# araju6/parameter-server-distributed

Hardware: AMD Instinct MI355X
Metric: samples/sec (whole node) ResNet-50 async-SGD (higher is better)
Workload: dtype bf16

## Files before the change

### parameter_server_distributed_amd/csrc/kernels/convn.hip

```cpp
#include "mfma_common.h"
#include "cu_count.h"
#include "launchers_convn.h"

namespace psd {

namespace {

constexpr int kBM = 128;
constexpr int kBK = 64;

__device__ __forceinline__ bf16x8 frag(const uint8_t* lds, int rb, int ks, int lane) {
  const int row = rb * 16 + (lane & 15);
  return __builtin_bit_cast(bf16x8, *reinterpret_cast<const u32x4*>(lds + kmaj_off(row, ks * 4 + (lane >> 4))));
}

template <int DPSK, int A, int OFF = 0>
__device__ __forceinline__ void wait_ahead(int ahead) {
  if constexpr (A <= 0) {
    wait_vm<OFF>();
  } else {
    if (ahead >= A) wait_vm<A * DPSK + OFF>();
    else wait_ahead<DPSK, A - 1, OFF>(ahead);
  }
}
// ... 835 lines not shown
        pf_at = T;
        __builtin_amdgcn_sched_barrier(0);
      } else {
        convn_epilogue<BM, BN, WNT, STATS, BWD, true>(a, acc, kshift, tile, wr, wc, lane, stg, pix, n0, es);
      }
#pragma unroll
      for (int i = 0; i < 4; ++i)
#pragma unroll
        for (int j = 0; j < G::JN; ++j) acc[i][j] = f32x4{0.f, 0.f, 0.f, 0.f};
    }
  }
  convn_flush<WNT, STATS, BWD>(a, es, (int64_t)blockIdx.x * G::WM + wr, wc, lane, n0);
}

__device__ __forceinline__ int hx_swz(int row) { return ((row >> 1) & 3) << 1; }
__device__ __forceinline__ int hx_off(int row, int kc) { return row * 128 + ((kc ^ hx_swz(row)) << 4); }

constexpr int kHxWin = 4 * 64 * 128;
constexpr int kHxW = 9 * 64 * 128;
constexpr int kHxLds = kHxW + 2 * kHxWin + 4 * 2048 + 512;

template <bool STATS, int BWD>
__global__ __launch_bounds__(256) void convh_kernel(ConvnArgs a, int ntiles) {
  extern __shared__ __attribute__((aligned(16))) uint8_t smem[];
  uint8_t* wlds = smem;
  auto winb = [&](int b) { return smem + kHxW + b * kHxWin; };
  const int lane = threadIdx.x & 63;
  const int wid = __builtin_amdgcn_readfirstlane(threadIdx.x >> 6);
  const int wr = wid >> 1, wc = wid & 1;
  const int cl = lane & 15;
  const int tpi = (a.Ho + 1) >> 1;
  const int t_begin = (int)(((int64_t)blockIdx.x * ntiles) / gridDim.x);
  const int t_end = (int)(((int64_t)(blockIdx.x + 1) * ntiles) / gridDim.x);
  if (t_begin >= t_end) return;
  float kshift[2] = {0.f, 0.f};
  if constexpr (STATS) {
#pragma unroll
    for (int j = 0; j < 2; ++j) kshift[j] = a.shift[wc * 32 + j * 16 + cl];
  }
  const rsrc_t xr = make_rsrc(a.x, a.xbytes);
  const rsrc_t wrs = make_rsrc(a.w, a.wbytes);
  for (int pc = wid; pc < 72; pc += 4) {
    const int t = pc >> 3, row = (pc & 7) * 8 + (lane >> 3);
    const int kc = (lane & 7) ^ hx_swz(row);
    const uint32_t off = ((uint32_t)row * (uint32_t)a.K + (uint32_t)(t * 64 + kc * 8)) * 2u;
    __builtin_amdgcn_raw_ptr_buffer_load_lds(wrs, (__attribute__((address_space(3))) void*)(wlds + pc * 1024), 16, off,
                                             0, 0, 0);
  }
  auto stage = [&](int tile, int b) {
    const int n = tile / tpi, ho0 = (tile - n * tpi) * 2;
#pragma unroll
    for (int i = 0; i < 8; ++i) {
      const int pc = i * 4 + wid;
      const int row = pc * 8 + (lane >> 3);
      const int jj = row >> 6, ws = row & 63;
      const int hi = ho0 - 1 + jj, wi = ws - 1;
      const int kc = (lane & 7) ^ hx_swz(row);
      const bool ok = (unsigned)hi < (unsigned)a.H && (unsigned)wi < (unsigned)a.W;
      const uint32_t off = ok ? ((((uint32_t)((n * a.H + hi) * a.W + wi)) << 6) + (uint32_t)(kc * 8)) * 2u : kOOB;
      __builtin_amdgcn_raw_ptr_buffer_load_lds(xr, (__attribute__((address_space(3))) void*)(winb(b) + pc * 1024), 16,
                                               off, 0, 0, 0);
    }
  };
  stage(t_begin, 0);
  wait_vm<0>();
  __syncthreads();
  uint8_t* stg = smem + kHxW + 2 * kHxWin + wid * 2048;
  EpiSums<2> es;
  es.zero();
  auto pix_of = [&](int tl) {
    const int n = tl / tpi, ho0 = (tl - n * tpi) * 2;
    return [=](int p) -> int {
      const int j = p >> 6, wo = p & 63;
      return ((wo < a.Wo) & (ho0 + j < a.Ho)) ? (n * a.Ho + ho0 + j) * a.Wo + wo : -1;
    };
  };
  for (int tile = t_begin, it = 0; tile < t_end; ++tile, ++it) {
    const int b = it & 1;
    if (tile + 1 < t_end) stage(tile + 1, b ^ 1);
    const uint8_t* win = winb(b);
    f32x4 acc[4][2];
#pragma unroll
    for (int i = 0; i < 4; ++i)
#pragma unroll
      for (int j = 0; j < 2; ++j) acc[i][j] = f32x4{0.f, 0.f, 0.f, 0.f};
    auto load_tap = [&](int tap, bf16x8 (&af)[2][4], bf16x8 (&bf)[2][2]) {
      const int tr = tap / 3, ts = tap - tr * 3;
      const uint8_t* Bs = wlds + tap * 8192;
#pragma unroll
      for (int ks = 0; ks < 2; ++ks) {
#pragma unroll
        for (int j = 0; j < 2; ++j)
          bf[ks][j] = __builtin_bit_cast(
              bf16x8, *reinterpret_cast<const u32x4*>(Bs + hx_off((wc * 2 + j) * 16 + (lane & 15), ks * 4 + (lane >> 4))));
#pragma unroll
        for (int i = 0; i < 4; ++i) {
          const int row = (wr + tr) * 64 + i * 16 + (lane & 15) + ts;
          af[ks][i] = __builtin_bit_cast(bf16x8, *reinterpret_cast<const u32x4*>(win + hx_off(row, ks * 4 + (lane >> 4))));
        }
      }
    };
    bf16x8 fa[2][2][4], fb[2][2][2];
    load_tap(0, fa[0], fb[0]);
#pragma unroll
    for (int tap = 0; tap < 9; ++tap) {
      const int cb = tap & 1;
      if (tap + 1 < 9) load_tap(tap + 1, fa[cb ^ 1], fb[cb ^ 1]);
      __builtin_amdgcn_sched_barrier(0);
#pragma unroll
      for (int ks = 0; ks < 2; ++ks)
#pragma unroll
        for (int i = 0; i < 4; ++i)
#pragma unroll
          for (int j = 0; j < 2; ++j)
            acc[i][j] = __builtin_amdgcn_mfma_f32_16x16x32_bf16(fa[cb][ks][i], fb[cb][ks][j], acc[i][j], 0, 0, 0);
      __builtin_amdgcn_sched_barrier(0);
    }
    wait_vm<0>();
    convn_epilogue<128, 64, 32, STATS, BWD, true>(a, acc, kshift, tile, wr, wc, lane, stg, pix_of(tile), 0, es);
    __syncthreads();
  }
  convn_flush<32, STATS, BWD>(a, es, (int64_t)blockIdx.x * 2 + wr, wc, lane, 0);
}

static bool convh_ok(const ConvnArgs& a) {
  return a.N == 64 && a.logC == 6 && a.R == 3 && a.S == 3 && a.stride == 1 && a.pad == 1 && a.H == a.Ho &&
         a.W == a.Wo && a.Wo + 2 <= 64 && !a.x2 && a.K == 576 && a.ldc == 64;
}

static int convh_grid(int ntiles) { return ntiles < cu_count() ? ntiles : cu_count(); }

template <bool STATS, int BWD>
static hipError_t convh_launch_t(const ConvnArgs& a, hipStream_t st) {
  static bool attr = false;
  if (!attr) {
    const hipError_t e =
        hipFuncSetAttribute((const void*)convh_kernel<STATS, BWD>, hipFuncAttributeMaxDynamicSharedMemorySize, kHxLds);
    if (e != hipSuccess) return e;
    attr = true;
  }
  const int ntiles = (a.M / (a.Ho * a.Wo)) * ((a.Ho + 1) / 2);
  hipLaunchKernelGGL((convh_kernel<STATS, BWD>), dim3(convh_grid(ntiles)), dim3(256), kHxLds, st, a, ntiles);
  return hipGetLastError();
}

static hipError_t convh_launch(const ConvnArgs& a, hipStream_t st) {
  if (a.bwd == 1) return convh_launch_t<false, 1>(a, st);
  if (a.bwd == 2) return convh_launch_t<false, 2>(a, st);
  if (a.bwd == 3) return convh_launch_t<false, 3>(a, st);
  if (a.bwd == 5) return convh_launch_t<false, 5>(a, st);
  return a.part ? convh_launch_t<true, 0>(a, st) : convh_launch_t<false, 0>(a, st);
}

template <int BN>
struct P1Cfg;
template <>
struct P1Cfg<256> {
  static constexpr int WNT = 64;
};
template <>
struct P1Cfg<128> {
  static constexpr int WNT = 32;
};
template <>
struct P1Cfg<64> {
  static constexpr int WNT = 32;
};
constexpr int kP1Slots = 3;
template <int BN>
constexpr int p1_lds() {
  using G = Geo<128, BN, P1Cfg<BN>::WNT, kP1Slots>;
  return kP1Slots * G::SLOT + G::NW * G::STG;
}

static int convp_grid_x(int tiles_m, int tiles_n) {
  int g = cu_count() / (tiles_n > 0 ? tiles_n : 1);
  if (g < 1) g = 1;
  return g < tiles_m ? g : tiles_m;
}

template <int BN>
static bool pf_ok(const ConvnArgs& a) {
  return BN == 256 && a.epi_prefetch && (a.bwd == 2 || a.bwd == 5 || a.bwd == 8) && a.ldc == a.N &&
         (int64_t)a.M * a.N * 2 <= 0xFFFFFF00ll && a.M < (1 << 24);
}

template <int BN, bool STATS, int BWD, bool PF = false, bool HASBX = true>
static hipError_t convp_launch_t(const ConvnArgs& a0, hipStream_t st, int grid_mul = 1) {
  constexpr int WNT = P1Cfg<BN>::WNT;
  using G = Geo<128, BN, WNT, kP1Slots>;
  constexpr int LDS = p1_lds<BN>();
  static_assert(LDS <= 160 * 1024, "LDS");
  static bool attr = false;
  if (!attr) {
    const hipError_t e = hipFuncSetAttribute((const void*)convp_kernel<BN, WNT, kP1Slots, STATS, BWD, PF, HASBX>,
                                             hipFuncAttributeMaxDynamicSharedMemorySize, LDS);
    if (e != hipSuccess) return e;
    attr = true;
  }
  ConvnArgs a = a0;
  a.nslot = kP1Slots;
  const int tiles_m = (a.M + 127) / 128, tiles_n = a.N / BN;
  int gx = convp_grid_x(tiles_m, tiles_n) * grid_mul;
  if (gx > tiles_m) gx = tiles_m;
  hipLaunchKernelGGL((convp_kernel<BN, WNT, kP1Slots, STATS, BWD, PF, HASBX>), dim3(gx, tiles_n), dim3(G::NT), LDS, st,
                     a, tiles_m);
  return hipGetLastError();
}

template <int BN>
static int pr_slots(int K) {
  using G = Geo<128, BN, P1Cfg<BN>::WNT, 3>;
  const int fixed = (K / kBK) * BN * 128 + G::NW * G::STG;
  int ns = (160 * 1024 - fixed) / (128 * 128);
  if (ns > kPrMaxSlots) ns = kPrMaxSlots;
  return ns >= 3 ? ns : 0;
}

template <int BN, bool STATS, int BWD, bool PF = false, bool HASBX = true>
static hipError_t convpr_launch_t(const ConvnArgs& a0, int ns, hipStream_t st, int grid_mul = 1) {
  constexpr int WNT = P1Cfg<BN>::WNT;
  using G = Geo<128, BN, WNT, 3>;
  static bool attr = false;
  if (!attr) {
    const hipError_t e = hipFuncSetAttribute((const void*)convpr_kernel<BN, WNT, STATS, BWD, PF, HASBX>,
                                             hipFuncAttributeMaxDynamicSharedMemorySize, 160 * 1024);
    if (e != hipSuccess) return e;
    attr = true;
  }
  ConvnArgs a = a0;
  a.nslot = ns;
  const int lds = (a.K / kBK) * BN * 128 + ns * 128 * 128 + G::NW * G::STG;
  const int tiles_m = (a.M + 127) / 128, tiles_n = a.N / BN;
  int gx = convp_grid_x(tiles_m, tiles_n) * grid_mul;
  if (gx > tiles_m) gx = tiles_m;
  hipLaunchKernelGGL((convpr_kernel<BN, WNT, STATS, BWD, PF, HASBX>), dim3(gx, tiles_n), dim3(G::NT), lds, st, a,
                     tiles_m);
  return hipGetLastError();
}

template <int BN>
static hipError_t convpr_launch_s(const ConvnArgs& a, int ns, hipStream_t st, int gm = 1) {
  if constexpr (BN == 256) {
    if (pf_ok<BN>(a)) {
      const bool hb = a.bx != nullptr;
      if (a.bwd == 2) return hb ? convpr_launch_t<BN, false, 2, true, true>(a, ns, st, gm)
                                : convpr_launch_t<BN, false, 2, true, false>(a, ns, st, gm);
      if (a.bwd == 5) return hb ? convpr_launch_t<BN, false, 5, true, true>(a, ns, st, gm)
                                : convpr_launch_t<BN, false, 5, true, false>(a, ns, st, gm);
      if (a.bwd == 8) return convpr_launch_t<BN, false, 8, true, true>(a, ns, st, gm);
    }
  }
  if (a.bwd == 1) return convpr_launch_t<BN, false, 1>(a, ns, st, gm);
  if (a.bwd == 2) return convpr_launch_t<BN, false, 2>(a, ns, st, gm);
  if (a.bwd == 3) return convpr_launch_t<BN, false, 3>(a, ns, st, gm);
  if (a.bwd == 5) return convpr_launch_t<BN, false, 5>(a, ns, st, gm);
  if (a.bwd == 8) return convpr_launch_t<BN, false, 8>(a, ns, st, gm);
  return a.part ? convpr_launch_t<BN, true, 0>(a, ns, st, gm) : convpr_launch_t<BN, false, 0>(a, ns, st, gm);
}

template <int BN>
static hipError_t convp_launch_s(const ConvnArgs& a, hipStream_t st, int gm = 1) {
  if (const int ns = pr_slots<BN>(a.K)) return convpr_launch_s<BN>(a, ns, st, gm);
  if constexpr (BN == 256) {
    if (pf_ok<BN>(a)) {
      const bool hb = a.bx != nullptr;
      if (a.bwd == 2) return hb ? convp_launch_t<BN, false, 2, true, true>(a, st, gm)
                                : convp_launch_t<BN, false, 2, true, false>(a, st, gm);
      if (a.bwd == 5) return hb ? convp_launch_t<BN, false, 5, true, true>(a, st, gm)
                                : convp_launch_t<BN, false, 5, true, false>(a, st, gm);
      if (a.bwd == 8) return convp_launch_t<BN, false, 8, true, true>(a, st, gm);
    }
  }
  if (a.bwd == 1) return convp_launch_t<BN, false, 1>(a, st, gm);
  if (a.bwd == 2) return convp_launch_t<BN, false, 2>(a, st, gm);
  if (a.bwd == 3) return convp_launch_t<BN, false, 3>(a, st, gm);
  if (a.bwd == 5) return convp_launch_t<BN, false, 5>(a, st, gm);
  if (a.bwd == 8) return convp_launch_t<BN, false, 8>(a, st, gm);
  return a.part ? convp_launch_t<BN, true, 0>(a, st, gm) : convp_launch_t<BN, false, 0>(a, st, gm);
}

template <int BN>
static hipError_t convp2_launch_s(const ConvnArgs& a, hipStream_t st) {
  using G = Geo<128, BN, P1Cfg<BN>::WNT, 3>;
  const int lds2 = (a.K / kBK) * BN * 128 + 2 * 128 * 128 + G::NW * G::STG;
  if (lds2 <= 80 * 1024) return convpr_launch_s<BN>(a, 2, st, 2);
  return convp_launch_s<BN>(a, st, 2);
}

static hipError_t convp2_launch(const ConvnArgs& a, int bn, hipStream_t st) {
  if (a.R != 1 || a.S != 1 || a.stride != 1 || a.pad != 0 || a.Ho != a.H || a.Wo != a.W) return hipErrorNotSupported;
  if (bn == 256) return convp2_launch_s<256>(a, st);
  if (bn == 128) return convp2_launch_s<128>(a, st);
  return convp2_launch_s<64>(a, st);
}

static hipError_t convp_launch(const ConvnArgs& a, int bn, hipStream_t st) {
  if (a.R != 1 || a.S != 1 || a.stride != 1 || a.pad != 0 || a.Ho != a.H || a.Wo != a.W) return hipErrorNotSupported;
  if (bn == 256) return convp_launch_s<256>(a, st);
  if (bn == 128) return convp_launch_s<128>(a, st);
  return convp_launch_s<64>(a, st);
}

template <int BM, int BN, int WNT, int NSLOT, bool STATS, int BWD>
static hipError_t convn_launch_t(const ConvnArgs& a0, hipStream_t st) {
  using G = Geo<BM, BN, WNT, NSLOT>;
  constexpr int LDS_MAX = NSLOT * G::SLOT + G::NW * G::STG;
  static_assert(LDS_MAX <= 160 * 1024, "LDS");
  static bool attr = false;
  if (!attr) {
    const hipError_t e = hipFuncSetAttribute((const void*)convn_kernel<BM, BN, WNT, NSLOT, STATS, BWD>,
                                             hipFuncAttributeMaxDynamicSharedMemorySize, LDS_MAX);
    if (e != hipSuccess) return e;
    attr = true;
  }
  ConvnArgs a = a0;
  const int nt = a.K / kBK;
  a.nslot = nt < NSLOT ? (nt < 2 ? 1 : nt) : NSLOT;
  const int lds = a.nslot * G::SLOT + G::NW * G::STG;
  const int tiles_m = (a.M + BM - 1) / BM;
  hipLaunchKernelGGL((convn_kernel<BM, BN, WNT, NSLOT, STATS, BWD>), dim3(tiles_m, a.N / BN), dim3(G::NT), lds, st, a);
  return hipGetLastError();
}

template <int BM, int BN, int WNT, int NSLOT>
static hipError_t convn_launch_s(const ConvnArgs& a, hipStream_t st) {
  if (a.bwd == 1) return convn_launch_t<BM, BN, WNT, NSLOT, false, 1>(a, st);
  if (a.bwd == 2) return convn_launch_t<BM, BN, WNT, NSLOT, false, 2>(a, st);
  if (a.bwd == 3) return convn_launch_t<BM, BN, WNT, NSLOT, false, 3>(a, st);
  if (a.bwd == 5) return convn_launch_t<BM, BN, WNT, NSLOT, false, 5>(a, st);
  if (a.bwd == 8) return convn_launch_t<BM, BN, WNT, NSLOT, false, 8>(a, st);
  return a.part ? convn_launch_t<BM, BN, WNT, NSLOT, true, 0>(a, st)
                : convn_launch_t<BM, BN, WNT, NSLOT, false, 0>(a, st);
}

int convn_tile_n(int N) {
  if (N == 64) return 64;
  if (N == 128) return 128;
  if (N % 256 == 0) return 256;
  return 0;
}

static int plain_count(int bn) { return bn == 256 ? 3 : 4; }
static int persist_count(int bn) { return bn == 64 ? 1 : 0; }
static int p1_count(int bn) { return bn ? 2 : 0; }
static int convn_variant_count(int bn) { return plain_count(bn) + persist_count(bn) + p1_count(bn); }
static bool is_persist(int bn, int v) { return v >= plain_count(bn) && v < plain_count(bn) + persist_count(bn); }
static bool is_p1(int bn, int v) { return v == plain_count(bn) + persist_count(bn); }
static bool is_p2(int bn, int v) { return v == plain_count(bn) + persist_count(bn) + 1; }

int convn_variant_kind(int N, int v) {
  const int bn = convn_tile_n(N);
  if (!bn || v < 0 || v >= convn_variant_count(bn)) return -1;
  return v < plain_count(bn) ? 0 : is_persist(bn, v) ? 2 : is_p1(bn, v) ? 3 : 4;
}

int convn_variants(int N) {
  const int bn = convn_tile_n(N);
  return bn ? convn_variant_count(bn) : 0;
}

static int default_variant(const ConvnArgs& a, int bn) {
  (void)a;
  (void)bn;
  return 0;
}

static int variant_bm(int bn, int v) {
  if (is_persist(bn, v) || is_p1(bn, v) || is_p2(bn, v)) return 128;
  if (bn == 64) return (v == 2 || v == 3) ? 256 : 128;
  if (bn == 128) return v == 2 ? 256 : 128;
  return 128;
}

bool convn_variant_ok(int N, int v, int R, int S, int stride, int pad, int Wo, bool has_x2) {
  const int bn = convn_tile_n(N);
  if (!bn || v < 0 || v >= convn_variant_count(bn)) return false;
  if (v < plain_count(bn)) return true;
  if (is_p1(bn, v) || is_p2(bn, v)) return R == 1 && S == 1 && stride == 1 && pad == 0;
  return !has_x2 && N == 64 && R == 3 && S == 3 && stride == 1 && pad == 1 && Wo + 2 <= 64;
}

int convn_stats_rows(int M) { return 4 * ((M + 255) / 256) + 4; }

int convn_part_rows_geo(int M, int N, int variant, int Ho, int Wo, int R) {
  const int bn = convn_tile_n(N);
  if (!bn) return 0;
  const int bm = variant_bm(bn, variant);
  if (is_persist(bn, variant)) {
    if (Ho <= 0 || Wo <= 0) return 0;
    return 2 * convh_grid((M / (Ho * Wo)) * ((Ho + 1) / 2));
  }
  if (is_p1(bn, variant)) return 2 * convp_grid_x((M + 127) / 128, N / bn);
  if (is_p2(bn, variant)) {
    const int t = (M + 127) / 128, g = 2 * convp_grid_x(t, N / bn);
    return 2 * (g < t ? g : t);
  }
  return (bm / 64) * ((M + bm - 1) / bm);
}

int convn_part_rows(int M, int N, int variant) { return convn_part_rows_geo(M, N, variant, 0, 0, 1); }

hipError_t launch_convn(const ConvnArgs& a_in, hipStream_t st) {
  if (a_in.M <= 0) return hipSuccess;
  ConvnArgs a = a_in;
  if (!a.x2) a.K1 = a.K;
  const int bn = convn_tile_n(a.N);
  const int C = 1 << a.logC;
  const bool two = a.x2 != nullptr;
  const int K1 = two ? a.K1 : a.K;
  const bool ok = bn > 0 && a.logC >= 6 && a.K % kBK == 0 && K1 == a.R * a.S * C && a.ldc % 8 == 0 &&
                  (!two || (a.R == 1 && a.S == 1 && a.stride == 1 && a.pad == 0 && a.logC2 >= 6 && K1 % kBK == 0 &&
                            a.K == K1 + (1 << a.logC2) && a.x2bytes > 0 && a.x2bytes <= 0xFFFFFF00u)) &&
                  a.ldc >= a.N && a.H < 32768 && a.W < 32768 && a.xbytes > 0 && a.xbytes <= 0xFFFFFF00u &&
                  a.wbytes > 0 && a.variant < convn_variant_count(bn) &&
                  (a.y || (a.bwd == 0 && a.part)) &&
                  (a.bwd == 0 ? (!a.part || a.shift)
                   : a.bwd == 8 ? (!a.part && a.bss && a.amask && a.ldc == a.N && a.N % 8 == 0)
                              : (a.part && (a.bx || a.bwd >= 2) && a.bmean && a.ldc == a.N &&
                                 (a.bwd == 1 ? a.bss != nullptr
                                             : ((a.bwd == 2 || a.bwd == 3 || a.bwd == 5) && a.bdr && a.bmbits &&
                                                (a.bwd != 3 || (a.bxd && a.bmean_d && a.part_d)) &&
                                                (a.bwd != 5 || (a.Ho % 2 == 0 && a.Wo % 2 == 0))))));
  if (!ok) return hipErrorNotSupported;
  if (a.ophase != 0 &&
      (a.ophase > 4 || a.variant < 0 || a.variant >= plain_count(bn) || two || a.stride != 1 || a.pad != 0 ||
       (a.bwd != 0 && a.bwd != 1) || a.M >= (1 << 24) || a.R > 2 || a.S > 2 ||
       (int64_t)a.M * 4 * a.ldc * 2 > 0x7FFFFFFFll))
    return hipErrorNotSupported;
  const int v = a.variant >= 0 ? a.variant : default_variant(a, bn);
  if (is_p1(bn, v)) return convp_launch(a, bn, st);
  if (is_p2(bn, v)) return convp2_launch(a, bn, st);
  if (is_persist(bn, v)) {
    if (!convh_ok(a) || a.bwd == 8 || !a.y) return hipErrorNotSupported;
    return convh_launch(a, st);
  }
  switch (bn) {
    case 64:
      if (v == 0) return convn_launch_s<128, 64, 32, 3>(a, st);
      if (v == 1) return convn_launch_s<128, 64, 32, 2>(a, st);
      if (v == 2) return convn_launch_s<256, 64, 64, 3>(a, st);
      return convn_launch_s<256, 64, 32, 3>(a, st);
    case 128:
      if (v == 0) return convn_launch_s<128, 128, 32, 3>(a, st);
      if (v == 1) return convn_launch_s<128, 128, 64, 3>(a, st);
      if (v == 2) return convn_launch_s<256, 128, 64, 2>(a, st);
      return convn_launch_s<128, 128, 32, 2>(a, st);
    default:
      if (v == 0) return convn_launch_s<128, 256, 64, 3>(a, st);
      if (v == 1) return convn_launch_s<128, 256, 64, 2>(a, st);
      return convn_launch_s<128, 128, 32, 2>(a, st);
  }
}

}
```

### parameter_server_distributed_amd/ops/conv.py

```python
from __future__ import annotations


import functools

import torch
import torch.nn as nn
import torch.nn.functional as F

from ..utils.config import feature as _feat
from . import wprep as _wprep
from . import autotune as _at
from .handover import (BwdPre, StatsPending, StridedDr, bn_momentum, fold_v as _fold_v, pop_dr, same, sinks, take,
                       take_dr)


def _enabled() -> bool:
    return _feat("conv1x1")


def _choose(key: tuple, candidates: dict) -> str:
    return _at.choose(("conv1x1",) + key, candidates, "miopen")


def decisions() -> dict:
# ... 5 lines not shown


def _native():
    from .. import native

    return native()


def _psd_ok(k: int, n: int) -> bool:
    return k % 8 == 0 and n % 8 == 0 and _feat("conv1x1_mfma")


def _as_2d(t: torch.Tensor) -> torch.Tensor:
    n, c, h, w = t.shape
    return t.permute(0, 2, 3, 1).reshape(n * h * w, c)


def _from_2d(t2: torch.Tensor, n: int, h: int, w: int) -> torch.Tensor:
    return t2.view(n, h, w, t2.shape[1]).permute(0, 3, 1, 2)


def _fp8_ok(k: int, n: int) -> bool:
    return k % 128 == 0 and k >= 256 and n >= 256 and n % 8 == 0 and _feat("fp8_compute")


def _q8(t2: torch.Tensor, e5m2: bool = False, scaler: "DelayedScale | None" = None):
    from . import quantize_fp8

    if scaler is not None:
        return scaler.quantize(t2, e5m2)
    return quantize_fp8(t2, e5m2=e5m2)


from .fp8_common import FP8_CALLS, mx_weight


def _mx_on() -> bool:
    return _feat("fp8_mx")


def _q_act(t: torch.Tensor, e5m2: bool = False, scaler: "DelayedScale | None" = None):
    if _mx_on():
        from . import quantize_mx

        return quantize_mx(t, e5m2=e5m2)
    return _q8(t, e5m2=e5m2, scaler=scaler)


def _q_weight(mod, w2: torch.Tensor):
    if _mx_on():
        return mx_weight(mod, w2)
    return _q8(w2)


def _take_dq8(mod, dy: torch.Tensor):
    return take(mod, "_psd_dq8_pending", dy, strides=True)


def _take_q8(mod, x: torch.Tensor):
    return take(mod, "_psd_q8_pending", x, strides=True)




def _psdn_ok(cin: int, cout: int) -> bool:
    return cin >= 64 and (cin & (cin - 1)) == 0 and (cout in (64, 128) or cout % 256 == 0) and \
        _feat("convn")


def _bn_consumer(mod):
    bn = getattr(mod, "_psd_bn", None) if mod is not None else None
    if bn is None or not bn.training or bn.running_mean is None or not _feat("convn_stats"):
        return None
    return bn


class _Lazy:
    __slots__ = ("fn", "t", "shape")

    def __init__(self, fn, shape):
        self.fn, self.t, self.shape = fn, None, tuple(shape)

    def __call__(self) -> torch.Tensor:
        if self.t is None:
            self.t = self.fn()
        return self.t


def _wt(w2: torch.Tensor, mod=None, weight=None) -> _Lazy:
    def make():
        t = _wprep.get(mod, weight, "t") if weight is not None else None
        return t if t is not None else w2.t().contiguous()
    return _Lazy(make, (w2.shape[1], w2.shape[0]))


def _wflip(mod, weight: torch.Tensor) -> torch.Tensor:
    t = _wprep.get(mod, weight, "f")
    if t is not None:
        return t
    cout, cin, k, _ = weight.shape
    return weight.flip(2, 3).permute(1, 2, 3, 0).reshape(cin, k * k * cout).contiguous()


def _get(w):
    return w() if isinstance(w, _Lazy) else w


def _out_hw(h: int, w: int, k: int, stride: int, pad: int) -> tuple:
    return (h + 2 * pad - k) // stride + 1, (w + 2 * pad - k) // stride + 1


def _convn_variants(x, w2, k: int, stride: int, pad: int, bn=None) -> dict:
    C = _native()
    n, _, h, w = x.shape
    cout = w2.shape[0]
    ho, wo = _out_hw(h, w, k, stride, pad)
    M = n * ho * wo

    def make(v, stats):
        def fn():
            out = torch.empty(M, cout, device=x.device, dtype=x.dtype)
            part = None
            if stats:
                part = torch.empty(_part_rows(M, cout, v, ho, wo, k), 2, cout, device=x.device, dtype=torch.float32)
            rows = C.convn_(x, _get(w2), out, k, k, stride, pad, part=part,
                            shift=bn.running_mean if stats else None, variant=v)
            if rows == 0:
                raise RuntimeError("convn_ declined a shape _psdn_ok accepted")
            y = _from_2d(out, n, ho, wo)
            if stats:
                bn._psd_stats_pending = StatsPending(y, part, rows)
            return y
        return fn

    ok = [v for v in range(C.convn_variants(cout)) if _variant_ok(cout, v, k, stride, pad, wo, x.shape[1], h)]
    cands = {f"psdn{v}": make(v, bn is not None) for v in ok}
    if bn is not None:
        cands.update({f"psdu{v}": make(v, False) for v in ok})
    return cands


def _variant_ok(cout: int, v: int, k: int, stride: int, pad: int, wo: int, cin: int | None = None,
                h: int | None = None) -> bool:
    C = _native()
    if not C.convn_variant_ok(cout, v, k, k, stride, pad, wo):
        return False
    kind = C.convn_variant_kind(cout, v)
    if kind == 2:
        return _feat("convn_persist") and cin == 64 and (h is None or h == wo)
    if kind == 3:
        return _feat("convn_p1")
    if kind == 4:
        return _feat("convn_p1") and _feat("convn_p2")
    return kind == 0


def _part_rows(M: int, N: int, v: int, ho: int, wo: int, k: int) -> int:
    C = _native()
    return max(C.convn_stats_rows(M), C.convn_part_rows(M, N, v, ho, wo, k))


def _fwd_records(ctx, mod) -> None:
    ctx.bn_in = getattr(mod, "_psd_bn_in", None) if mod is not None else None
    ctx.strided_to = getattr(mod, "_psd_strided_to", None) if mod is not None else None


def _bn_bwd_fusion(bn, x: torch.Tensor):
    st = getattr(bn, "_psd_fwd", None) if bn is not None else None
    if st is None or not _feat("convn_bwd"):
        return None
    y, bx, mean, ss, mbits, xd, mean_d = st
    if not same(y, x, strides=True):
        return None
    if mbits is not None:
        if not bn._psd_pending_dr:
            return None
        if isinstance(bn._psd_pending_dr[-1], StridedDr):
            if xd is not None or x.shape[2] % 2 or x.shape[3] % 2 or not _feat("convn_bwd5"):
                return None
            return dict(mode=5, bn=bn, bx=bx, mean=mean, mbits=mbits)
        if xd is not None:
            if not _feat("convn_bwd3"):
                return None
            return dict(mode=3, bn=bn, bx=bx, mean=mean, mbits=mbits, bxd=xd, mean_d=mean_d)
        return dict(mode=2, bn=bn, bx=bx, mean=mean, mbits=mbits)
    return dict(mode=1, bn=bn, bx=bx, mean=mean, ss=ss)


def _take_dr_for(fu) -> None:
    if fu is not None:
        fu["dr"] = fu["bn"]._psd_pending_dr.pop() if fu["mode"] >= 2 else None


def _convn_bwd_launch(dy, w2, cout: int, k: int, pad: int, v: int, fu: dict, prows: int, declined: str,
                      x2=None, bias=None) -> torch.Tensor:
    n, _, h, w = dy.shape
    out = torch.empty(n * h * w, cout, device=dy.device, dtype=dy.dtype)
    part = torch.empty(prows, 2, cout, device=dy.device, dtype=torch.float32)
    part_d = torch.empty_like(part) if fu["mode"] == 3 else None
    rows = _native().convn_bwd_(dy, w2, out, k, k, 1, pad, part, v, fu["mode"], fu["bx"], fu["mean"],
                                bss=fu.get("ss"), bdr=_dr_arg(fu.get("dr")), bmbits=fu.get("mbits"), x2=x2,
                                bias=bias, bxd=fu.get("bxd"), bmean_d=fu.get("mean_d"), part_d=part_d,
                                epi_prefetch=_feat("convp_epi_prefetch"))
    if rows == 0:
        raise RuntimeError(declined)
    g = _from_2d(out, n, h, w)
    fu["bn"]._psd_bwd_pre = BwdPre(g, part, rows, part_d)
    return g


def _convn_bwd_variants(dy, w2, k: int, pad: int, fu: dict) -> dict:
    C = _native()
    n, _, h, w = dy.shape
    cout = w2.shape[0]

    def make(v):
        return lambda: _convn_bwd_launch(dy, _get(w2), cout, k, pad, v, fu, _part_rows(n * h * w, cout, v, h, w, k) + 1,
                                         "convn_bwd_ declined a shape _psdn_ok accepted")

    return {f"psdnb{v}": make(v) for v in range(C.convn_variants(cout))
            if _variant_ok(cout, v, k, 1, pad, w, dy.shape[1], h)}


def _s2_phase_weights(weight: torch.Tensor) -> list:
    cin = weight.shape[1]
    sel = (lambda t, d: t.narrow(d, 1, 1), lambda t, d: t[(slice(None),) * d + (slice(None, None, 2),)].flip(d))
    out = []
    for ph in (0, 1):
        for pw in (0, 1):
            wsel = sel[pw](sel[ph](weight, 2), 3)
            out.append(wsel.permute(1, 2, 3, 0).reshape(cin, -1).contiguous())
    return out


def _dgrad_s2_phases(dy, weight, x, fu, mod=None) -> dict:
    C = _native()
    n, cin, h, w = x.shape
    ho, wo = dy.shape[2], dy.shape[3]
    def phases():
        got = _wprep.get(mod, weight, "p")
        return got if got is not None else _s2_phase_weights(weight)

    wph = _Lazy(phases, (4,))

    def make(v, fused):
        def fn():
            out = torch.empty(n * h * w, cin, device=dy.device, dtype=dy.dtype)
            if fused:
                part = torch.empty(C.convn_dgrad_s2_rows(n, ho, wo, cin, v) + 1, 2, cin, device=dy.device,
                                   dtype=torch.float32)
                rows = C.convn_dgrad_s2_(dy, wph(), out, v, part=part, bx=fu["bx"], bmean=fu["mean"], bss=fu["ss"])
            else:
                rows = C.convn_dgrad_s2_(dy, wph(), out, v)
            if rows == 0:
                raise RuntimeError("convn_dgrad_s2_ declined a shape it was offered for")
            g = _from_2d(out, n, h, w)
            if fused:
                fu["bn"]._psd_bwd_pre = BwdPre(g, part, rows)
            return g
        return fn

    cands = {}
    for v in range(C.convn_variants(cin)):
        if C.convn_variant_kind(cin, v) != 0 or not C.convn_variant_ok(cin, v, 2, 2, 1, 0, wo, False):
            continue
        cands[f"psdns{v}"] = make(v, False)
        if fu is not None:
            cands[f"psdnbs{v}"] = make(v, True)
    return cands


def _dgrad_route(key: tuple, cands: dict, default: str, fu, dy_like, timed=None, defer=None):
    timed = cands if timed is None else timed
    if fu is None:
        how = _at.choose(key, timed, default)
        return cands[how]() if how != defer else None
    if fu.get("bx") is None:
        cands = {name: fn for name, fn in cands.items() if name.startswith("psdnb")}
        if not cands:
            raise RuntimeError("psd: a BN without its stored input needs the fused bwd-data epilogue")
        key, default = key + ("nobx",), next(iter(cands))
    timed = {n: (timed[n] if n.startswith("psdnb") else _with_bn_bwd_reduce(timed[n], fu)) for n in cands}
    how = _at.choose(key + ("bnbwd",), timed, default, group=lambda n: n.startswith("psdnb"))
    out = cands[how]() if how != defer else None
    if not how.startswith("psdnb"):
        fu["bn"]._psd_bwd_pre = None
        if fu.get("dr") is not None:
            fu["bn"]._psd_pending_dr.append(fu["dr"])
    return out


def _with_bn_reduce(fn, bn):
    def g():
        y = fn()
        _native().bn_reduce_(y, bn.running_mean)
        return y
    return g


def _with_bn_bwd_reduce(fn, fu):
    def g():
        dx = fn()
        _native().bn_bwd_reduce_(dx, fu["bx"], fu["mean"], ss=fu.get("ss"), dy2=take_dr(fu.get("dr")),
                                 mbits=fu.get("mbits"))
        return dx
    return g


def _stats_part(bn, M: int, cout: int, device):
    if bn is None or not _feat("gemm_stats"):
        return None
    return torch.empty(_native().gemm_stats_rows(M), 2, cout, device=device, dtype=torch.float32)


def _hand_stats(bn, y, part, rows: int):
    if part is not None and rows > 0:
        bn._psd_stats_pending = StatsPending(y, part, rows)


def _dr_arg(dr):
    return dr.t4 if isinstance(dr, StridedDr) else dr


def _route(key: tuple, cands: dict, default: str, bn=None) -> str:
    if bn is None:
        return _at.choose(key, cands, default)
    timed = {name: (fn if name.startswith(("psdn", "psds")) else _with_bn_reduce(fn, bn))
             for name, fn in cands.items()}
    how = _at.choose(key + ("bnstats",), timed, default)
    bn._psd_stats_pending = None
    return how


def _convw_cands(dy, x, k: int, stride: int, pad: int) -> dict:
    if not _feat("convw"):
        return {}
    C = _native()
    cout, cin = dy.shape[1], x.shape[1]
    kk = k * k * cin
    if cin < 64 or (cin & (cin - 1)) or not (cout in (64, 128) or cout % 256 == 0):
        return {}

    def make(v):
        def fn(into=None):
            o = into if into is not None else torch.empty(cout, kk, device=dy.device, dtype=dy.dtype)
            if not C.convw_(dy, x, o, k, k, stride, pad, variant=v):
                raise _at.Declined(f"convw_ variant {v}")
            return o.view(cout, k, k, cin).permute(0, 3, 1, 2)
        return fn

    nv = C.convw_variants(cout, kk)
    persist = 1 if (cout == 64 and kk == 576) else 0
    shapes = (nv - persist) // 2
    vs = [v for v in range(nv) if (v < shapes or _feat("convw_twostage")) and (v < 2 * shapes or _feat("convw_persist"))]
    return {f"psdw{v}": make(v) for v in vs}


class DelayedScale:

    def __init__(self, margin: float = 1.0):
        self.margin = float(margin)
        self.hist = None

    def quantize(self, x: torch.Tensor, e5m2: bool):
        from . import FP8_E4M3_MAX, FP8_E5M2_MAX, quantize_fp8

        x = x.contiguous()
        if self.hist is None or self.hist.device != x.device or not _feat("fp8_delayed"):
            q, sinv = quantize_fp8(x, e5m2=e5m2)
            if _feat("fp8_delayed"):
                self.hist = torch.zeros(2, dtype=torch.float32, device=x.device)
                self.hist[:1].copy_(sinv * (FP8_E5M2_MAX if e5m2 else FP8_E4M3_MAX) / self.margin)
            return q, sinv
        q = torch.empty(x.shape, dtype=torch.float8_e5m2 if e5m2 else torch.float8_e4m3fn, device=x.device)
# ... 588 lines not shown
```

### parameter_server_distributed_amd/utils/config.py

```python
from __future__ import annotations

import argparse
import json
import os


def load_config(path: str) -> dict:
    with open(path) as f:
        text = f.read()
    if path.endswith(".json"):
        cfg = json.loads(text)
    else:
        import yaml

        cfg = yaml.safe_load(text) or {}
    if not isinstance(cfg, dict):
        raise ValueError(f"{path}: a run config must be a mapping of option -> value")
    return {str(k).replace("-", "_"): v for k, v in cfg.items()}


def apply_config(ap: argparse.ArgumentParser, argv: list[str] | None = None) -> None:
    pre = argparse.ArgumentParser(add_help=False)
    pre.add_argument("--config", default=os.environ.get("PSD_CONFIG", ""))
    known, _ = pre.parse_known_args(argv)
    if not any(a.dest == "config" for a in ap._actions):
        ap.add_argument("--config", default="", help="YAML/JSON run config (flags override it)")
    if not known.config:
        return
    cfg = load_config(known.config)
    dests = {a.dest for a in ap._actions}
    unknown = sorted(set(cfg) - dests)
    if unknown:
        raise SystemExit(f"{known.config}: unknown option(s) {unknown}")
    ap.set_defaults(**cfg)


FEATURES: dict[str, tuple[bool, str]] = {
    "conv1x1": (True, "per-shape routing of 1x1 convolutions (MIOpen / hipBLASLt / MFMA); off: MIOpen only"),
    "conv1x1_mfma": (True, "the 8-phase MFMA GEMM as a 1x1-convolution candidate"),
    "conv_igemm": (True, "implicit-GEMM MFMA convolution (gemm.hip) as a forward / bwd-data candidate"),
    "conv_wgrad": (True, "implicit-GEMM MFMA weight gradient as a candidate"),
    "convn": (True, "narrow implicit-GEMM convolution kernels (convn.hip) as candidates"),
    "convn_stats": (True, "consumer-BN statistics in the narrow convolution's epilogue"),
    "convn_persist": (True, "persistent layer-1 3x3 kernel (convh)"),
    "convn_p1": (True, "persistent 1x1 kernels (convp / convpr)"),
    "convn_p2": (True, "the persistent 1x1 kernel at two workgroups per CU (two-slot ring) as a candidate"),
    "convp_epi_prefetch": (True, "persistent 1x1 kernels, 256-wide tiles, epilogue modes 2 / 5 / 8: the epilogue "
                                 "operands (dr / residual, mask bytes, BN input) loaded one tile ahead; off: loaded "
                                 "at the top of each tile's epilogue (same results bit for bit, "
                                 "profiles/convp_epi_prefetch.md)"),
    "convn_bwd": (True, "producing BN's backward reduction in the bwd-data epilogue (modes 1/2)"),
    "convn_bwd3": (True, "the dual-BN tail's reduction in the bwd-data epilogue (mode 3)"),
    "convn_bwd5": (True, "stride-2 downsample gradient added on the quarter grid (mode 5)"),
    "dgrad_s2_phase": (True, "stride-2 3x3 bwd-data as four output-parity phase launches of the narrow kernel "
                              "(with the producing BN's backward reduction in the epilogue) vs MIOpen"),
    "convw": (True, "narrow weight-gradient kernel (convw.hip) as a candidate"),
    "convw_persist": (True, "persistent layer-1 3x3 weight gradient (convhw)"),
    "convw_twostage": (True, "narrow weight-gradient tiles also on a two-stage ring at two workgroups per CU"),
    "convw_fold2": (True, "the BN-fold and Gram weight-gradient launches on the two-stage ring (two workgroups per CU)"),
    "gemm_stats": (True, "consumer-BN statistics in the 8-phase GEMM epilogue"),
    "library_candidates": (False, "convolutions: autotune also times MIOpen / hipBLASLt candidates wherever one of "
                                  "our kernels takes the shape; off (default): our kernels only there, the library "
                                  "only as the fallback -- same-box ResNet-50 15,681 / 15,695 vs 15,557 / 15,591 "
                                  "img/s with them (profiles/r6/ab_library_candidates.md)"),
    "library_linear": (True, "Linear layers: hipBLASLt stays an autotune candidate (BERT-base same-box 9,576 / 9,505 "
                             "vs 9,297 / 9,362 seq/s without it: it wins the QKV forward, the attention-output "
                             "bwd-data and the MLM-head weight gradient in the step, profiles/r6/ab_library_candidates.md)"),
    "prefer_own": (True, "autotune: our kernel takes a pick a library candidate wins by < 2 % (ops/autotune.py OWN_MARGIN)"),
    "wprep": (True, "every convolution's bwd-data weight operand (transpose / tap flip / stride-2 phases) in one batched launch per step (ops/wprep.py)"),
    "bn_fold": (True, "bn3's backward folded into conv3's bwd-data / weight-gradient GEMMs"),
    "bn_fold_ds": (True, "the stride-1 downsample BN folded into its convolution's backward"),
    "dual_nobx": (True, "downsample blocks' dual tail without the BN inputs in the consumer epilogue"),
    "tail_recompute": (True, "identity blocks' conv3 output recomputed instead of stored"),
    "tail_gram": (True, "the recomputing tail's statistics from the Gram matrix of conv3's input"),
    "dual_recompute": (True, "stride-1 downsample blocks: neither conv3's nor the downsample conv's output stored"),
    "fp8_compute": (True, "fp8 convolutions / Linear layers where the model asks for them"),
    "fp8_mx": (True, "MX block scales for every fp8 operand; off: per-tensor scales"),
    "fp8_mx_handover": (True, "BN passes write the consumer's MX e4m3 input / producer's MX e5m2 dY"),
    "fp8_delayed": (True, "per-tensor fp8: delayed (previous-call amax) scaling"),
    "fp8_dgrad": (True, "fp8 e5m2-dY bwd-data of the fp8 convolutions and fp8 Linear layers"),
    "fp8_wgrad": (False, "fp8 e4m3 x e4m3 split-K weight gradient of the fp8 Linear layers (tokens % 128 == 0); off: bf16"),
    "fp8_ln_handover": (True, "the fused LayerNorm writes the MX e4m3 input of the fp8 Linear that consumes it"),
    "async_cached_local": (True, "async PS at world 1: inbox / publish buffers in plain (cached) device memory "
                                 "instead of uncached IPC memory (AsyncPS hands it to the native engine)"),
    "async_apply_background": (True, "async PS with SSP bound >= 1: the owner's apply on a normal-priority stream "
                                     "with at most 512 workgroups, beside the compute stream (AsyncPS hands it to "
                                     "the native engine); off: high priority, full grid (the S = 0 setting)"),
    "async_direct_pull": (True, "async PS at world 1: each step pulls straight into the model's working weights "
                                "on the compute stream (one local copy) instead of prefetching into a second "
                                "buffer and copying that into the working weights"),
    "tail_fp8": (False, "fp8 models' identity blocks: conv3 + bn3 as the bf16 recomputing tail (bn3 folded "
                       "into conv3's bf16 backward, conv3's output never stored); read at model build. Off: same-box "
                       "WRN-101-2 4,136 vs 4,170 img/s (profiles/r6/ab_tail_fp8.md)"),
    "linear_tune": (True, "per-shape MFMA / hipBLASLt choice for Linear layers; off: MFMA only"),
    "gelu_fuse": (True, "GELU backward in the consumer Linear's bwd-data GEMM epilogue"),
    "attn_bias": (True, "QKV bias gradient handed over by the attention backward"),
    "attn_long": (True, "streaming fused attention kernels for S = 192 .. 512 (multiples of 64); off: SDPA on "
                        "transposed views there, as for every other S > 128"),
    "attn_xlong": (True, "the streaming fused attention kernels also at S = 576 .. 4096 (multiples of 64; needs "
                         "attn_long); off: S > 512 goes back to SDPA on transposed views"),
    "rope": (True, "in-place rotary position embedding kernel on the packed QKV (ops/rope.py RotaryQK); off: the "
                   "out-of-place torch composite rope_ref"),
    "rmsnorm": (True, "fused residual add + dropout + RMSNorm kernels (ops/rmsnorm.py FusedAddRMSNorm); off: the "
                      "torch composite add_rmsnorm_ref"),
    "swiglu": (True, "gated SiLU kernels on the packed gate/up tensor (ops/swiglu.py SwiGLU); off: the torch "
                     "composite swiglu_ref"),
}

_FEAT_ENV: str | None = None
_FEAT_OVR: dict[str, bool] = {}
_FEAT_SET: dict[str, bool] = {}


def _feature_env() -> dict[str, bool]:
    global _FEAT_ENV, _FEAT_OVR
    raw = os.environ.get("PSD_FEATURES", "")
    if raw != _FEAT_ENV:
        ovr = {}
        for item in filter(None, (t.strip() for t in raw.split(","))):
            name, _, val = item.partition("=")
            name = name.strip()
            if name not in FEATURES:
                raise ValueError(f"PSD_FEATURES: unknown feature {name!r} (known: {sorted(FEATURES)})")
            ovr[name] = val.strip() not in ("0", "false", "off", "no")
        _FEAT_ENV, _FEAT_OVR = raw, ovr
    return _FEAT_OVR


def feature(name: str) -> bool:
    if name in _FEAT_SET:
        return _FEAT_SET[name]
    ovr = _feature_env()
    if name in ovr:
        return ovr[name]
    return FEATURES[name][0]


def set_feature(name: str, on: bool | None) -> None:
    if name not in FEATURES:
        raise ValueError(f"unknown feature {name!r}")
    if on is None:
        _FEAT_SET.pop(name, None)
    else:
        _FEAT_SET[name] = bool(on)


def features() -> dict[str, bool]:
    return {n: feature(n) for n in FEATURES}


FAULTS: dict[str, tuple[int, str]] = {
    "stop_heartbeat_after": (-1, "worker: stop sending coordinator heartbeats after n of them"),
    "push_delay_ms": (0, "worker: sleep this long before every gradient push"),
    "exit_after_push": (-1, "worker: exit the process right after its k-th push"),
    "selftest_fail_rank": (-1, "async PS: this rank reports a failed start-up self-test"),
    "selftest_fail_kernel": (-1, "async PS: this rank fails the kernel-transport self-test attempt only"),
}


def fault(name: str) -> int:
    if name not in FAULTS:
        raise ValueError(f"unknown fault key {name!r}")
    for item in filter(None, (t.strip() for t in os.environ.get("PSD_FAULT", "").split(","))):
        k, _, v = item.partition("=")
        if k.strip() == name:
            return int(v)
    return FAULTS[name][0]
```

Before: 16880.

## Add persistent window-based 3x3 conv kernel as autotune candidate for wide channels

Adds a persistent 512-thread 3x3 stride-1 convolution kernel. It stages a haloed input window in LDS once per tile and channel block, then reuses it across all nine taps, while weight slices stream through a three-slot ring. The point is to cut the redundant input reloads of the im2col-style narrow kernel for the 128- to 512-channel layers. It is registered as a new variant kind, enabled by default, that the autotuner can pick. It adds a large LDS footprint (one workgroup per CU) and a new epilogue path that has to be correct for the stats and bwd modes.

```diff
diff --git a/parameter_server_distributed_amd/csrc/kernels/convn.hip b/parameter_server_distributed_amd/csrc/kernels/convn.hip
--- a/parameter_server_distributed_amd/csrc/kernels/convn.hip
+++ b/parameter_server_distributed_amd/csrc/kernels/convn.hip
@@ -1011,6 +1011,213 @@
   return a.part ? convh_launch_t<true, 0>(a, st) : convh_launch_t<false, 0>(a, st);
 }
 
+constexpr int kWnWin = 384 * 128;
+constexpr int kWnW = 128 * 128;
+constexpr int kWnLds = 2 * kWnWin + 3 * kWnW + 8 * 2048;
+static_assert(kWnLds <= 160 * 1024, "LDS");
+__device__ __forceinline__ void wn_wait(int k) {
+  static_assert(2 + 2 < 64, "vmcnt is 6 bits");
+  if (k <= 1) wait_vm<2>();
+  else if (k == 2 || k == 8) wait_vm<3>();
+  else wait_vm<4>();
+}
+
+struct WnBlk {
+  int ct, tl, cb;
+};
+
+template <bool STATS, int BWD>
+__global__ __launch_bounds__(512) void convwin_kernel(ConvnArgs a, int ntiles, int lsw) {
+  constexpr int WNT = 64, JN = 4;
+  extern __shared__ __attribute__((aligned(16))) uint8_t smem[];
+  auto winb = [&](int b) { return smem + b * (kWnWin + kWnW); };
+  auto wslot = [&](int s) { return smem + (s == 0 ? kWnWin : 2 * kWnWin + s * kWnW); };
+  const int lane = threadIdx.x & 63;
+  const int wid = __builtin_amdgcn_readfirstlane(threadIdx.x >> 6);
+  const int wr = wid >> 1, wc = wid & 1;
+  const int cl = lane & 15;
+  const int SW = 1 << lsw, RT = 256 >> lsw;
+  const int tpi = (a.Ho + RT - 1) >> (8 - lsw);
+  const int gx = gridDim.x;
+  const int bq = xcd_remap(blockIdx.x, gx);
+  const int t_begin = (int)(((int64_t)bq * ntiles) / gx);
+  const int t_end = (int)(((int64_t)(bq + 1) * ntiles) / gx);
+  const int ntl = t_end - t_begin;
+  if (ntl <= 0) return;
+  const int ncb = (1 << a.logC) >> 6, nct = a.N >> 7;
+  const int nblk = nct * ntl * ncb;
+  const rsrc_t xr = make_rsrc(a.x, a.xbytes);
+  const rsrc_t wrs = make_rsrc(a.w, a.wbytes);
+
+  auto next_blk = [&](WnBlk b) {
+    if (++b.cb == ncb) {
+      b.cb = 0;
+      if (++b.tl == ntl) {
+        b.tl = 0;
+        ++b.ct;
+      }
+    }
+    return b;
+  };
+  auto stage_w = [&](const WnBlk& b, int tap, bool live, int s) {
+    uint8_t* slot = wslot(s);
+    const int k0 = (tap << a.logC) + b.cb * 64;
+#pragma unroll
+    for (int i = 0; i < 2; ++i) {
+      const int piece = i * 8 + wid;
+      const int row = piece * 8 + (lane >> 3);
+      const int kc = (lane & 7) ^ ((row >> 1) & 7);
+      const uint32_t off = live ? ((uint32_t)(b.ct * 128 + row) * (uint32_t)a.K + (uint32_t)(k0 + kc * 8)) * 2u : kOOB;
+      __builtin_amdgcn_raw_ptr_buffer_load_lds(wrs, (__attribute__((address_space(3))) void*)(slot + piece * 1024), 16,
+                                               off, 0, 0, 0);
+    }
+  };
+  auto stage_win = [&](const WnBlk& b, int i, bool live, int wb) {
+    const int tile = t_begin + b.tl;
+    const int n = tile / tpi, ho0 = (tile - n * tpi) * RT;
+    const int pc = i * 8 + wid;
+    const int q = pc * 8 + (lane >> 3);
+    const int jj = q >> lsw, ws = q & (SW - 1);
+    const int hi = ho0 - 1 + jj, wi = ws - 1;
+    const int kc = (lane & 7) ^ hx_swz(q);
+    const bool ok = live && jj < RT + 2 && (unsigned)hi < (unsigned)a.H && (unsigned)wi < (unsigned)a.W;
+    const uint32_t off =
+        ok ? ((((uint32_t)((n * a.H + hi) * a.W + wi)) << a.logC) + (uint32_t)(b.cb * 64 + kc * 8)) * 2u : kOOB;
+    __builtin_amdgcn_raw_ptr_buffer_load_lds(xr, (__attribute__((address_space(3))) void*)(winb(wb) + pc * 1024), 16, off,
+                                             0, 0, 0);
+  };
+
+  float kshift[JN];
+#pragma unroll
+  for (int j = 0; j < JN; ++j) kshift[j] = 0.f;
+  if constexpr (STATS) {
+#pragma unroll
+    for (int j = 0; j < JN; ++j) kshift[j] = a.shift[wc * WNT + j * 16 + cl];
+  }
+  WnBlk cur{0, 0, 0};
+  WnBlk nxt = next_blk(cur);
+  __builtin_amdgcn_sched_barrier(0);
+#pragma unroll
+  for (int i = 0; i < 6; ++i) stage_win(cur, i, true, 0);
+  stage_w(cur, 0, true, 0);
+  stage_w(cur, 1, true, 1);
+  __builtin_amdgcn_sched_barrier(0);
+
+  int aoff[3][2];
+#pragma unroll
+  for (int ts = 0; ts < 3; ++ts)
+#pragma unroll
+    for (int ks = 0; ks < 2; ++ks) aoff[ts][ks] = hx_off(cl + ts, ks * 4 + (lane >> 4));
+
+  f32x4 acc[4][JN];
+#pragma unroll
+  for (int i = 0; i < 4; ++i)
+#pragma unroll
+    for (int j = 0; j < JN; ++j) acc[i][j] = f32x4{0.f, 0.f, 0.f, 0.f};
+  EpiSums<JN> es;
+  es.zero();
+  uint8_t* stg = smem + 2 * kWnWin + 3 * kWnW + wid * 2048;
+
+  for (int B = 0; B < nblk; ++B) {
+    const bool nlive = B + 1 < nblk;
+    const uint8_t* win = winb(B & 1) + wr * 64 * 128;
+#pragma unroll
+    for (int k = 0; k < 9; ++k) {
+      wn_wait(k);
+      __builtin_amdgcn_s_barrier();
+      __builtin_amdgcn_sched_barrier(0);
+      if (k + 2 < 9) stage_w(cur, k + 2, true, (k + 2) % 3);
+      else stage_w(nxt, k + 2 - 9, nlive, (k + 2) % 3);
+      if (k >= 1 && k <= 6) stage_win(nxt, k - 1, nlive, (B + 1) & 1);
+      const int tr = k / 3, ts = k - tr * 3;
+      const uint8_t* As = win + ((tr << lsw) << 7);
+      const uint8_t* Bs = wslot(k % 3);
+      bf16x8 af[2][4], bf[2][JN];
+#pragma unroll
+      for (int ks = 0; ks < 2; ++ks) {
+#pragma unroll
+        for (int j = 0; j < JN; ++j) bf[ks][j] = frag(Bs, wc * JN + j, ks, lane);
+#pragma unroll
+        for (int i = 0; i < 4; ++i)
+          af[ks][i] = __builtin_bit_cast(bf16x8, *reinterpret_cast<const u32x4*>(As + aoff[ts][ks] + i * 2048));
+      }
+#pragma unroll
+      for (int ks = 0; ks < 2; ++ks)
+#pragma unroll
+        for (int i = 0; i < 4; ++i)
+#pragma unroll
+          for (int j = 0; j < JN; ++j)
+            acc[i][j] = __builtin_amdgcn_mfma_f32_16x16x32_bf16(af[ks][i], bf[ks][j], acc[i][j], 0, 0, 0);
+      __builtin_amdgcn_sched_barrier(0);
+    }
+    if (cur.cb == ncb - 1) {
+      const int tile = t_begin + cur.tl;
+      const int n = tile / tpi, ho0 = (tile - n * tpi) * RT;
+      const int n0 = cur.ct * 128;
+      const int pbase = (n * a.Ho + ho0) * a.Wo;
+      const int jlim = a.Ho - ho0;
+      auto pix = [&](int p) -> int {
+        const int j = p >> lsw, wo = p & (SW - 1);
+        return ((wo < a.Wo) & (j < jlim)) ? ((pbase + (int)__umul24((unsigned)j, (unsigned)a.Wo) + wo) & 0x7FFFFFFF) : -1;
+      };
+      __builtin_assume(a.y != nullptr);
+      convn_epilogue<256, 128, WNT, STATS, BWD, true>(a, acc, kshift, tile, wr, wc, lane, stg, pix, n0, es);
+#pragma unroll
+      for (int i = 0; i < 4; ++i)
+#pragma unroll
+        for (int j = 0; j < JN; ++j) acc[i][j] = f32x4{0.f, 0.f, 0.f, 0.f};
+      if (cur.tl == ntl - 1) {
+        convn_flush<WNT, STATS, BWD>(a, es, (int64_t)bq * 4 + wr, wc, lane, n0);
+        es.zero();
+        if constexpr (STATS) {
+          if (nlive) {
+#pragma unroll
+            for (int j = 0; j < JN; ++j) kshift[j] = a.shift[nxt.ct * 128 + wc * WNT + j * 16 + cl];
+          }
+        }
+      }
+      __builtin_amdgcn_sched_barrier(0);
+    }
+    cur = nxt;
+    nxt = next_blk(nxt);
+  }
+}
+
+static int convwin_lsw(int Wo) { return Wo + 2 <= 16 ? 4 : Wo + 2 <= 32 ? 5 : 6; }
+
+static int convwin_tiles(int M, int Ho, int Wo) {
+  const int rt = 256 >> convwin_lsw(Wo);
+  return (M / (Ho * Wo)) * ((Ho + rt - 1) / rt);
+}
+
+static int convwin_grid(int ntiles) { return ntiles < cu_count() ? ntiles : cu_count(); }
+
+static bool convwin_ok(const ConvnArgs& a) {
+  return a.N % 128 == 0 && a.logC >= 6 && a.R == 3 && a.S == 3 && a.stride == 1 && a.pad == 1 && a.H == a.Ho &&
+         a.W == a.Wo && a.Wo + 2 <= 64 && !a.x2 && a.K == (9 << a.logC) && a.ophase == 0 && a.y &&
+         (a.bwd == 0 || a.bwd == 1) && (int64_t)a.N * a.K * 2 <= 0xFFFFFF00ll;
+}
+
+template <bool STATS, int BWD>
+static hipError_t convwin_launch_t(const ConvnArgs& a, hipStream_t st) {
+  static bool attr = false;
+  if (!attr) {
+    const hipError_t e =
+        hipFuncSetAttribute((const void*)convwin_kernel<STATS, BWD>, hipFuncAttributeMaxDynamicSharedMemorySize, kWnLds);
+    if (e != hipSuccess) return e;
+    attr = true;
+  }
+  const int ntiles = convwin_tiles(a.M, a.Ho, a.Wo);
+  hipLaunchKernelGGL((convwin_kernel<STATS, BWD>), dim3(convwin_grid(ntiles)), dim3(512), kWnLds, st, a, ntiles,
+                     convwin_lsw(a.Wo));
+  return hipGetLastError();
+}
+
+static hipError_t convwin_launch(const ConvnArgs& a, hipStream_t st) {
+  if (a.bwd == 1) return convwin_launch_t<false, 1>(a, st);
+  return a.part ? convwin_launch_t<true, 0>(a, st) : convwin_launch_t<false, 0>(a, st);
+}
+
 template <int BN>
 struct P1Cfg;
 template <>
@@ -1203,15 +1410,17 @@
 static int plain_count(int bn) { return bn == 256 ? 3 : 4; }
 static int persist_count(int bn) { return bn == 64 ? 1 : 0; }
 static int p1_count(int bn) { return bn ? 2 : 0; }
-static int convn_variant_count(int bn) { return plain_count(bn) + persist_count(bn) + p1_count(bn); }
+static int win_count(int bn) { return bn == 128 || bn == 256 ? 1 : 0; }
+static int convn_variant_count(int bn) { return plain_count(bn) + persist_count(bn) + p1_count(bn) + win_count(bn); }
 static bool is_persist(int bn, int v) { return v >= plain_count(bn) && v < plain_count(bn) + persist_count(bn); }
 static bool is_p1(int bn, int v) { return v == plain_count(bn) + persist_count(bn); }
 static bool is_p2(int bn, int v) { return v == plain_count(bn) + persist_count(bn) + 1; }
+static bool is_win(int bn, int v) { return win_count(bn) && v == plain_count(bn) + persist_count(bn) + 2; }
 
 int convn_variant_kind(int N, int v) {
   const int bn = convn_tile_n(N);
   if (!bn || v < 0 || v >= convn_variant_count(bn)) return -1;
-  return v < plain_count(bn) ? 0 : is_persist(bn, v) ? 2 : is_p1(bn, v) ? 3 : 4;
+  return v < plain_count(bn) ? 0 : is_persist(bn, v) ? 2 : is_p1(bn, v) ? 3 : is_p2(bn, v) ? 4 : 5;
 }
 
 int convn_variants(int N) {
@@ -1237,6 +1446,7 @@
   if (!bn || v < 0 || v >= convn_variant_count(bn)) return false;
   if (v < plain_count(bn)) return true;
   if (is_p1(bn, v) || is_p2(bn, v)) return R == 1 && S == 1 && stride == 1 && pad == 0;
+  if (is_win(bn, v)) return !has_x2 && R == 3 && S == 3 && stride == 1 && pad == 1 && Wo + 2 <= 64;
   return !has_x2 && N == 64 && R == 3 && S == 3 && stride == 1 && pad == 1 && Wo + 2 <= 64;
 }
 
@@ -1249,6 +1459,10 @@
   if (is_persist(bn, variant)) {
     if (Ho <= 0 || Wo <= 0) return 0;
     return 2 * convh_grid((M / (Ho * Wo)) * ((Ho + 1) / 2));
+  }
+  if (is_win(bn, variant)) {
+    if (Ho <= 0 || Wo <= 0 || R != 3 || Wo + 2 > 64) return 0;
+    return 4 * convwin_grid(convwin_tiles(M, Ho, Wo));
   }
   if (is_p1(bn, variant)) return 2 * convp_grid_x((M + 127) / 128, N / bn);
   if (is_p2(bn, variant)) {
@@ -1294,6 +1508,7 @@
     if (!convh_ok(a) || a.bwd == 8 || !a.y) return hipErrorNotSupported;
     return convh_launch(a, st);
   }
+  if (is_win(bn, v)) return convwin_ok(a) ? convwin_launch(a, st) : hipErrorNotSupported;
   switch (bn) {
     case 64:
       if (v == 0) return convn_launch_s<128, 64, 32, 3>(a, st);
diff --git a/parameter_server_distributed_amd/ops/conv.py b/parameter_server_distributed_amd/ops/conv.py
--- a/parameter_server_distributed_amd/ops/conv.py
+++ b/parameter_server_distributed_amd/ops/conv.py
@@ -181,6 +181,8 @@
         return _feat("convn_p1")
     if kind == 4:
         return _feat("convn_p1") and _feat("convn_p2")
+    if kind == 5:
+        return _feat("convn_window") and (h is None or h == wo)
     return kind == 0
 
 
@@ -248,7 +250,8 @@
                                          "convn_bwd_ declined a shape _psdn_ok accepted")
 
     return {f"psdnb{v}": make(v) for v in range(C.convn_variants(cout))
-            if _variant_ok(cout, v, k, 1, pad, w, dy.shape[1], h)}
+            if _variant_ok(cout, v, k, 1, pad, w, dy.shape[1], h)
+            and (C.convn_variant_kind(cout, v) != 5 or fu["mode"] == 1)}
 
 
 def _s2_phase_weights(weight: torch.Tensor) -> list:
diff --git a/parameter_server_distributed_amd/utils/config.py b/parameter_server_distributed_amd/utils/config.py
--- a/parameter_server_distributed_amd/utils/config.py
+++ b/parameter_server_distributed_amd/utils/config.py
@@ -43,6 +43,8 @@
     "convn": (True, "narrow implicit-GEMM convolution kernels (convn.hip) as candidates"),
     "convn_stats": (True, "consumer-BN statistics in the narrow convolution's epilogue"),
     "convn_persist": (True, "persistent layer-1 3x3 kernel (convh)"),
+    "convn_window": (True, "persistent window 3x3 kernel for the 128- to 512-channel convolutions (convwin) as a "
+                           "candidate (profiles/convn_window.md)"),
     "convn_p1": (True, "persistent 1x1 kernels (convp / convpr)"),
     "convn_p2": (True, "the persistent 1x1 kernel at two workgroups per CU (two-slot ring) as a candidate"),
     "convp_epi_prefetch": (True, "persistent 1x1 kernels, 256-wide tiles, epilogue modes 2 / 5 / 8: the epilogue "
```

Result: no change. 17010, median of 6 (+0.8%).
